# toposware/certificate-stark

Hardware: AMD Instinct MI355X
Metric: proofs/sec, state_transition AIR @ 2^20 steps (complete prove(): trace gen, LDE, Blake3 commitments, constraint evaluation, composition, DEEP, FRI, 96 queries) (higher is better)
Workload: dtype u64 (63-bit prime field, Montgomery) + u32 (Blake3)

## Files before the change

certificate-stark_amd/csrc/rounds_layout.h:

```cpp
#pragma once
#include "constraints.h"
#include "mds_mfma.cuh"

namespace cs {

struct RoundWindow { int reg, res_a, flag_a, res_b, flag_b; };
#define CS_ROUND_WINDOWS_INIT {{0, 0, 3, 0, -1}, {15, 14, 0, 15, 1}, {29, 28, 0, 29, 1}, {44, 42, 0, 44, 1}, {42, 42, 2, 0, -1}}
#define CS_WINDOW_GROUPS_INIT {{{0, 1, -1}, {-1, -1, -1}}, {{1, 2, 0}, {1, 2, 0}}, {{0, 2, -1}, {0, 2, -1}}, {{2, -1, -1}, {2, -1, -1}}, {{2, -1, -1}, {-1, -1, -1}}}

constexpr int RT_SECTIONS = 5 * 2 * 4;
constexpr int RT_A = 0, RT_UL = RT_SECTIONS * 64, RT_ML = RT_UL + RT_SECTIONS * 14 * 2, RT_MT = RT_ML + 14 * 14 * 2;
constexpr size_t MT_BYTES = (mdsmfma::table_bytes(14) + 15) & ~(size_t)15;
constexpr int RT_G = RT_MT + (int)(MT_BYTES / 8);
constexpr int RT_MF = (RT_G + RT_SECTIONS * 14 + 1) & ~1;

constexpr int MF_TILES_INV = 7, MF_TILES_SEC = 13, MF_KS_INV = 4, MF_KS_SEC = 7;
constexpr int MF_INV_D = RT_MF;
constexpr int MF_SEC_D = MF_INV_D + MF_TILES_INV * 4 * 8;
constexpr int MF_K = MF_SEC_D + MF_TILES_SEC * 4 * 16;
constexpr int RT_SIZE = MF_K + (14 + 2 * MF_TILES_SEC) * 4;
constexpr int RT_LAM = RT_SIZE;
static_assert(RT_LAM + CE_GFOLD_WORDS <= CE_RTAB_WORDS, "rtab size");
__host__ __device__ constexpr int mf_tile_base(int w) { return w == 0 ? 0 : w == 1 ? 2 : w == 2 ? 6 : w == 3 ? 10 : w == 4 ? 12 : 13; }
__host__ __device__ constexpr int mf_tile_window(int t) { return t < 2 ? 0 : t < 6 ? 1 : t < 10 ? 2 : t < 12 ? 3 : 4; }
__host__ __device__ constexpr int mf_tile_fs(int w, int local) { return (w == 1 || w == 2) ? local >> 1 : w == 3 ? local : 0; }
__host__ __device__ constexpr int mf_tile_pair(int w, int local) { return (w == 1 || w == 2) ? local & 1 : w == 0 ? local : 0; }

constexpr int MR_SECTIONS = 8, MR_A = 0, MR_UL = MR_SECTIONS * 64, MR_ML = MR_UL + MR_SECTIONS * 14 * 2, MR_G = MR_ML + 196 * 2;
constexpr int MRF_INV_D = MR_G + MR_SECTIONS * 14;
constexpr int MRF_SEC_D = MRF_INV_D + MF_TILES_INV * 32;
constexpr int MRF_K = MRF_SEC_D + 4 * 64;
constexpr int MR_SIZE = MRF_K + (14 + 8) * 4;
static_assert(MR_SIZE <= MERKLE_RTAB_LAMBDA, "MerkleAir rounds table");

hipError_t launch_merkle_rounds_mfma(const AirCombineParams &p, const uint64_t *ptab, uint64_t *d_rtab, unsigned nk, unsigned round_group, int which,
                                     hipStream_t stream);
hipError_t launch_rounds_mfma(const CeParams &p, uint64_t *d_even, hipStream_t stream);

}
```

certificate-stark_amd/csrc/rounds_mfma.hip:

```cpp
#include "rounds_layout.h"
#include "rescue.cuh"

namespace cs {
namespace {

using mdsmfma::v16i;
using mdsmfma::v4i;
typedef unsigned __int128 u128;

#ifndef RM_NT_
#define RM_NT_ 256
#endif
#ifndef RM_WAVES
#define RM_WAVES 2
#endif
constexpr int RM_NT = RM_NT_;
template <int PTS> constexpr int rw_rows = 32 * PTS + 2;
template <int PTS> constexpr int rw_img = 14 * rw_rows<PTS>;
constexpr uint64_t X0 = mdsmfma::X0;
constexpr uint64_t HALF_P = (FP_P - 1) / 2;
enum { P_SETUP = 0, P_HASH = 4, P_SCHNORR_HASH = 12, P_ARK = 20 };

__constant__ RoundWindow c_windows[5] = CS_ROUND_WINDOWS_INIT;
__constant__ int c_window_groups[5][2][3] = CS_WINDOW_GROUPS_INIT;

__device__ inline uint64_t digit_word(int64_t v) {
    uint64_t w = 0;
    int carry = 0;
    for (int a = 0; a < 8; a++) {
        int b = (a < 7 ? (int)(((uint64_t)v >> (8 * a)) & 0xff) : (int)(v >> 56)) + carry;
        carry = (a < 7 && b >= 128) ? 1 : 0;
        w |= (uint64_t)(uint8_t)(int8_t)(b - 256 * carry) << (8 * a);
    }
    return w;
}
__device__ __forceinline__ u128 acc0_offset() {
    u128 off = 0;
    for (int d = 0; d < 15; d++) off += (u128)mdsmfma::ACC0 << (8 * d);
    return off;
}

__device__ inline void build_inverse_tile(int T, int t, uint64_t *d_out, uint64_t *k_out) {
    if (t < 32) {
        const int g = t >> 4, h = (t >> 3) & 1, m = t & 7, i = 2 * T + g, j = 4 * (m >> 1) + 2 * h + (m & 1);
        d_out[(g * 2 + h) * 8 + m] = j < 14 ? digit_word((int64_t)c_inv_mds[i * 14 + j]) : 0;
    } else if (t < 34) {
        const int i = 2 * T + (t - 32);
        u128 k = 0;
        for (int j = 0; j < 14; j++) k += (u128)c_inv_mds[i * 14 + j] * X0;
        k -= acc0_offset();
        for (int q = 0; q < 4; q++) k_out[4 * (t - 32) + q] = (uint32_t)(k >> (32 * q));
    }
}
__device__ inline void build_section_tile(const fp *gam0, const fp *gam1, const uint32_t *ul0, const uint32_t *ul1, int t, uint64_t *d_out,
                                          uint64_t *k_out, fp (*csum)[32]) {
    if (t < 56) {
        const int g = t / 28, h = (t / 14) & 1, m = t % 14;
        fp c;
        if (m < 7) c = (g ? gam1 : gam0)[2 * m + h];
        else {
            const uint32_t *l = (g ? ul1 : ul0) + (2 * (m - 7) + h) * 4;
            c = fp_neg((fp)l[0] | ((fp)l[1] << 21) | ((fp)l[2] << 42));
        }
        d_out[(g * 2 + h) * 16 + m] = digit_word(c > HALF_P ? (int64_t)(c - FP_P) : (int64_t)c);
        csum[g][h * 14 + m] = c;
    } else {
        const int q = t - 56;
        d_out[(q >> 1) * 16 + 14 + (q & 1)] = 0;
    }
    __syncthreads();
    if (t < 2) {
        fp sum = 0;
        for (int e = 0; e < 28; e++) sum = fp_add(sum, csum[t][e]);
        const fp kc = fp_mul(fp_mul(X0 + HALF_P, sum), FP_R2);
        u128 k = (u128)kc + ((u128)(2 * FP_P) << 64);
        k -= acc0_offset();
        for (int q = 0; q < 4; q++) k_out[4 * t + q] = (uint32_t)(k >> (32 * q));
    }
}

__global__ void k_rounds_mfma_tables(fp *__restrict__ rtab) {
    rtab += (size_t)blockIdx.y * CE_RTAB_WORDS;
    const int t = threadIdx.x;
    if (blockIdx.x < MF_TILES_INV) {
        build_inverse_tile(blockIdx.x, t, rtab + MF_INV_D + blockIdx.x * 32, rtab + MF_K + 8 * blockIdx.x);
        return;
    }
    const int tile = blockIdx.x - MF_TILES_INV, w = mf_tile_window(tile), local = tile - mf_tile_base(w);
    const int sec = (w * 2 + mf_tile_fs(w, local)) * 4 + 2 * mf_tile_pair(w, local);
    __shared__ fp csum[2][32];
    const uint32_t *ul = (const uint32_t *)(rtab + RT_UL);
    build_section_tile(rtab + RT_G + sec * 14, rtab + RT_G + (sec + 1) * 14, ul + sec * 56, ul + (sec + 1) * 56, t, rtab + MF_SEC_D + tile * 64,
                       rtab + MF_K + 4 * (14 + 2 * tile), csum);
}
__global__ void k_merkle_rounds_mfma_tables(fp *__restrict__ rtab) {
    const int t = threadIdx.x;
    if (blockIdx.x < MF_TILES_INV) {
        build_inverse_tile(blockIdx.x, t, rtab + MRF_INV_D + blockIdx.x * 32, rtab + MRF_K + 8 * blockIdx.x);
        return;
    }
    const int w = blockIdx.x - MF_TILES_INV;
    __shared__ fp csum[2][32];
    const uint32_t *ul = (const uint32_t *)(rtab + MR_UL);
    build_section_tile(rtab + MR_G + (2 * w) * 14, rtab + MR_G + (2 * w + 1) * 14, ul + (2 * w) * 56, ul + (2 * w + 1) * 56, t, rtab + MRF_SEC_D + w * 64,
                       rtab + MRF_K + 4 * (14 + 2 * w), csum);
}

typedef __attribute__((address_space(3))) void lds_void;
typedef const __attribute__((address_space(1))) void glb_void;
template <int PTS>
__device__ __forceinline__ void fetch_window(const fp *rows, size_t n, int reg, int lane, fp *img) {
    if (lane < 16 * PTS + 1) {
#pragma unroll
        for (int j = 0; j < 14; j++)
            __builtin_amdgcn_global_load_lds((glb_void *)(rows + (size_t)(reg + j) * n), (lds_void *)(img + j * rw_rows<PTS>), 16, 0, 0);
    }
}
__device__ __forceinline__ v4i pack2(uint64_t a, uint64_t b) {
    v4i r;
    r[0] = (int)(uint32_t)a; r[1] = (int)(uint32_t)(a >> 32); r[2] = (int)(uint32_t)b; r[3] = (int)(uint32_t)(b >> 32);
    return r;
}
__device__ __forceinline__ v4i expand_frag(uint64_t d0, uint64_t d1, uint32_t sel_lo, uint32_t sel_hi) {
    v4i r;
    r[0] = (int)__builtin_amdgcn_perm((uint32_t)(d0 >> 32), (uint32_t)d0, sel_lo);
    r[1] = (int)__builtin_amdgcn_perm((uint32_t)(d0 >> 32), (uint32_t)d0, sel_hi);
    r[2] = (int)__builtin_amdgcn_perm((uint32_t)(d1 >> 32), (uint32_t)d1, sel_lo);
    r[3] = (int)__builtin_amdgcn_perm((uint32_t)(d1 >> 32), (uint32_t)d1, sel_hi);
    return r;
}
__device__ __forceinline__ v16i acc_start() {
    v16i a;
#pragma unroll
    for (int v = 0; v < 16; v++) a[v] = mdsmfma::ACC0;
    return a;
}
template <uint32_t V>
__device__ __forceinline__ uint32_t opaque_const() {
    uint32_t r;
    asm("s_mov_b32 %0, %1" : "=s"(r) : "n"(V));
    return r;
}
struct Shifts { uint32_t one, s8, s16, s24; };
__device__ __forceinline__ fp recombine_mad(const v16i &acc, const uint64_t (&k)[4], const Shifts &c) {
#ifdef RM_OLD_RECOMBINE
    return mdsmfma::recombine(acc, k[0] | (k[1] << 32), k[2] | (k[3] << 32));
#endif
    uint64_t s[4];
#pragma unroll
    for (int q = 0; q < 4; q++) {
        uint64_t t = mad_u64_u32((uint32_t)acc[4 * q], c.one, k[q]);
        t = mad_u64_u32((uint32_t)acc[4 * q + 1], c.s8, t);
        t = mad_u64_u32((uint32_t)acc[4 * q + 2], c.s16, t);
        if (4 * q + 3 < 15) t = mad_u64_u32((uint32_t)acc[4 * q + 3], c.s24, t);
        s[q] = t;
    }
    unsigned cy;
    const uint32_t w0 = (uint32_t)s[0];
    const uint32_t w1 = __builtin_addc((uint32_t)(s[0] >> 32), (uint32_t)s[1], 0u, &cy);
    const uint32_t w2 = __builtin_addc((uint32_t)(s[1] >> 32), (uint32_t)s[2], cy, &cy);
    const uint32_t w3 = (uint32_t)(s[2] >> 32) + (uint32_t)s[3] + cy;
    Acc128 a{((uint64_t)w1 << 32) | w0, ((uint64_t)w3 << 32) | w2};
    acc_fold(a);
    return acc_reduce(a);
}
#ifndef RM_DBUF
#define RM_DBUF 0
#endif
#ifndef RM_RESIDENT_
#define RM_RESIDENT_ 4096
#endif
constexpr unsigned RM_RESIDENT = RM_RESIDENT_;

struct Role {
    int lane, nn, h, ag;
    uint32_t sel_lo, sel_hi;
};
__device__ __forceinline__ void frag_selectors(int d, uint32_t &lo, uint32_t &hi) {
    lo = hi = 0;
#pragma unroll
    for (int b = 0; b < 4; b++) {
        const int a0 = d - b, a1 = d - 4 - b;
        lo |= (uint32_t)((a0 >= 0 && a0 <= 7 && d < 15) ? a0 : 0x0c) << (8 * b);
        hi |= (uint32_t)((a1 >= 0 && a1 <= 7 && d < 15) ? a1 : 0x0c) << (8 * b);
    }
}
__device__ __forceinline__ Role make_role(int lane) {
    Role r;
    r.lane = lane; r.nn = lane & 31; r.h = lane >> 5; r.ag = (r.nn >> 2) & 1;
    frag_selectors((r.nn & 3) + 4 * (r.nn >> 3), r.sel_lo, r.sel_hi);
    return r;
}
__device__ __forceinline__ void expand_inverse_table(v4i *inv_lds, const uint64_t *inv_d, int tid, int nthreads) {
    for (unsigned e = tid; e < MF_TILES_INV * MF_KS_INV * 64; e += nthreads) {
        const unsigned l = e & 63, ts = e >> 6, r = l & 31, hh = l >> 5, g = (r >> 2) & 1;
        uint32_t slo, shi;
        frag_selectors((int)((r & 3) + 4 * (r >> 3)), slo, shi);
        const uint64_t *dw = inv_d + ((ts >> 2) * 4 + g * 2 + hh) * 8 + 2 * (ts & 3);
        inv_lds[e] = expand_frag(dw[0], dw[1], slo, shi);
    }
}
template <int PTS, int DBUF>
__device__ __forceinline__ void window_operands(const fp *imgA, const fp *ark2, const v4i *inv_lds, const uint64_t *k_lds, const Role &ro,
                                                const Shifts &sh, v4i (&c)[PTS][MF_KS_SEC]) {
    constexpr int RWR = rw_rows<PTS>;
    const int h = ro.h, lane = ro.lane;
    v4i b[PTS][MF_KS_INV];
#pragma unroll
    for (int s = 0; s < MF_KS_INV; s++) {
        const int jb = (s == 3 && h) ? 12 : 4 * s + 2 * h;
        const fp k0 = ark2[jb], k1 = ark2[jb + 1];
#pragma unroll
        for (int pt = 0; pt < PTS; pt++)
            b[pt][s] = pack2(fp_sub(imgA[jb * RWR + 32 * pt + 1], k0) ^ X0, fp_sub(imgA[(jb + 1) * RWR + 32 * pt + 1], k1) ^ X0);
    }
    uint64_t held[PTS];
    auto inv_tile = [&](int T, v16i (&a)[PTS]) {
#pragma unroll
        for (int pt = 0; pt < PTS; pt++) a[pt] = acc_start();
#pragma unroll
        for (int s = 0; s < MF_KS_INV; s++) {
            const v4i fr = inv_lds[(T * MF_KS_INV + s) * 64 + lane];
#pragma unroll
            for (int pt = 0; pt < PTS; pt++) a[pt] = __builtin_amdgcn_mfma_i32_32x32x32_i8(fr, b[pt][s], a[pt], 0, 0, 0);
        }
    };
    auto finish_tile = [&](int T, const v16i (&a)[PTS]) {
        const uint64_t *kp = k_lds + 4 * (2 * T + h);
        const uint64_t kw[4] = {kp[0], kp[1], kp[2], kp[3]};
#pragma unroll
        for (int pt = 0; pt < PTS; pt++) {
            const uint64_t x = (fp_cube(recombine_mad(a[pt], kw, sh)) - HALF_P) ^ X0;
            if (T & 1) c[pt][T >> 1] = pack2(held[pt], x);
            else held[pt] = x;
        }
    };
    if constexpr (DBUF > 0) {
        v16i acc[2][PTS];
        inv_tile(0, acc[0]);
#pragma unroll
        for (int T = 0; T < MF_TILES_INV; T++) {
            if (T + 1 < MF_TILES_INV) inv_tile(T + 1, acc[(T + 1) & 1]);
            finish_tile(T, acc[T & 1]);
            if (T + 1 < MF_TILES_INV) {
#pragma unroll
                for (int e = 0; e < 4 * PTS; e++) {
                    __builtin_amdgcn_sched_group_barrier(0x008, 1, 0);
                    __builtin_amdgcn_sched_group_barrier(0x002, DBUF, 0);
                }
            }
        }
    } else {
#pragma unroll
        for (int T = 0; T < MF_TILES_INV; T++) {
            v16i acc[PTS];
            inv_tile(T, acc);
            finish_tile(T, acc);
        }
    }
#pragma unroll
    for (int t = 0; t < 7; t++) {
#pragma unroll
        for (int pt = 0; pt < PTS; pt++) {
            const uint64_t x = (fp_cube(imgA[(2 * t + h) * RWR + 32 * pt]) - HALF_P) ^ X0;
            if (t & 1) held[pt] = x;
            else c[pt][3 + (t >> 1)] = pack2(held[pt], x);
        }
    }
}
template <int PTS>
__device__ __forceinline__ void section_tile(const uint64_t *tile_d, const uint64_t *kp, const Role &ro, const Shifts &sh, const v4i (&c)[PTS][MF_KS_SEC],
                                             fp (&r)[PTS]) {
    v16i a[PTS];
#pragma unroll
    for (int pt = 0; pt < PTS; pt++) a[pt] = acc_start();
    const uint64_t *dw = tile_d + (ro.ag * 2 + ro.h) * 16;
#pragma unroll
    for (int s = 0; s < MF_KS_SEC; s++) {
        const v4i fr = expand_frag(dw[2 * s], dw[2 * s + 1], ro.sel_lo, ro.sel_hi);
#pragma unroll
        for (int pt = 0; pt < PTS; pt++) a[pt] = __builtin_amdgcn_mfma_i32_32x32x32_i8(fr, c[pt][s], a[pt], 0, 0, 0);
    }
    const uint64_t kw[4] = {kp[0], kp[1], kp[2], kp[3]};
#pragma unroll
    for (int pt = 0; pt < PTS; pt++) r[pt] = recombine_mad(a[pt], kw, sh);
}
__device__ __forceinline__ fp other_half(fp v) {
    const uint32_t lo = __shfl_xor((uint32_t)v, 32), hi = __shfl_xor((uint32_t)(v >> 32), 32);
    return ((uint64_t)hi << 32) | lo;
}

#ifndef RM_DBUF1
#define RM_DBUF1 0
#endif
#ifndef RM_PTS
#define RM_PTS 2
#endif
constexpr size_t RM_LDS_INV = (size_t)MF_TILES_INV * MF_KS_INV * 64 * 16;
template <int PTS, int NT = RM_NT> constexpr size_t rm_lds_img = (size_t)(NT / 64) * rw_img<PTS> * 8;
constexpr size_t RM_LDS_SEC = (size_t)MF_TILES_SEC * 4 * 16 * 8;
constexpr size_t RM_LDS_KINV = 14 * 32, RM_LDS_KSEC = (size_t)2 * MF_TILES_SEC * 32;
constexpr size_t RM_LDS_ARK = 8 * 14 * 8, RM_LDS_ATAB = (size_t)2 * MF_TILES_SEC * 8 * 8;
template <int PTS, int M, int NT> constexpr size_t rm_lds = RM_LDS_INV + rm_lds_img<PTS, NT> + RM_LDS_KINV + RM_LDS_ARK + M * (RM_LDS_SEC + RM_LDS_KSEC + RM_LDS_ATAB);

template <int PTS, int M, int NT>
__global__ __launch_bounds__(NT, PTS == 1 ? 3 : RM_WAVES) void k_rounds_mfma(CeParams p, fp *__restrict__ out) {
    constexpr int RWR = rw_rows<PTS>, WROWS = 32 * PTS, BROWS = NT / 64 * WROWS;
    constexpr int RM_NT = NT;
    extern __shared__ __attribute__((aligned(16))) uint8_t lds[];
    v4i *inv_lds = (v4i *)lds;
    fp *img_all = (fp *)(lds + RM_LDS_INV);
    uint64_t *kinv_lds = (uint64_t *)(lds + RM_LDS_INV + rm_lds_img<PTS, NT>);
    fp *ark2_lds = kinv_lds + RM_LDS_KINV / 8;
    uint64_t *secd_lds = ark2_lds + RM_LDS_ARK / 8;
    uint64_t *ksec_lds = secd_lds + M * (RM_LDS_SEC / 8);
    fp *atab_lds = ksec_lds + M * (RM_LDS_KSEC / 8);

    const size_t n = (size_t)1 << p.log_n;
    const unsigned kk = 2 * blockIdx.y, kc = (p.k0 >> 1) + blockIdx.y, ka = 2 * kc;
    const int tid = threadIdx.x, lane = tid & 63;
    const Role ro = make_role(lane);
    const int nn = ro.nn, h = ro.h;
    const fp *rt = p.rtab;
    expand_inverse_table(inv_lds, rt + MF_INV_D, tid, RM_NT);
    for (unsigned e = tid; e < RM_LDS_KINV / 8; e += RM_NT) kinv_lds[e] = rt[MF_K + e];
    for (unsigned e = tid; e < M * (RM_LDS_SEC / 8); e += RM_NT) secd_lds[e] = rt[(size_t)(e / (RM_LDS_SEC / 8)) * CE_RTAB_WORDS + MF_SEC_D + e % (RM_LDS_SEC / 8)];
    for (unsigned e = tid; e < M * (RM_LDS_KSEC / 8); e += RM_NT) ksec_lds[e] = rt[(size_t)(e / (RM_LDS_KSEC / 8)) * CE_RTAB_WORDS + MF_K + 14 * 4 + e % (RM_LDS_KSEC / 8)];
    if (tid < 8 * 14) {
        const unsigned r = tid / 14, c = tid % 14;
        ark2_lds[tid] = p.ptab[((size_t)ka * 48 + P_ARK + 14 + c) * 1024 + r];
    }
    for (unsigned e = tid; e < M * 2 * MF_TILES_SEC * 8; e += RM_NT) {
        const int c = e / (2 * MF_TILES_SEC * 8), r = e % (2 * MF_TILES_SEC * 8), tile = r >> 4, g = (r >> 3) & 1, w = mf_tile_window(tile), local = tile - mf_tile_base(w);
        const int sec = (w * 2 + mf_tile_fs(w, local)) * 4 + 2 * mf_tile_pair(w, local) + g;
        atab_lds[e] = rt[(size_t)c * CE_RTAB_WORDS + RT_A + sec * 64 + ka * 8 + (r & 7)];
    }
    __syncthreads();

    fp *img = img_all + (size_t)(tid >> 6) * rw_img<PTS>;
    const uint64_t *k_lds = kinv_lds;
    const fp *imgA = img + nn;
    const unsigned jrp = (unsigned)(nn & 7);
    const fp *ark2 = ark2_lds + jrp * 14;
    const fp *per = p.ptab + (size_t)(p.k0 + kk) * 48 * 1024;
    const fp *colbase = p.lde + (size_t)kk * 94 * n;
    const Shifts sh{opaque_const<1>(), opaque_const<1u << 8>(), opaque_const<1u << 16>(), opaque_const<1u << 24>()};
    const size_t nblk = n / BROWS;
    size_t blk = blockIdx.x;
    auto rows_of = [&](size_t b) {
        const size_t jw = b * (size_t)BROWS + (size_t)(tid >> 6) * WROWS;
        return colbase + jw + 2 * lane - ((lane == 16 * PTS && jw + WROWS == n) ? n : 0);
    };
    const fp *rows = rows_of(blk);
    if (blk < nblk) fetch_window<PTS>(rows, n, c_windows[0].reg, lane, img);
#pragma unroll 1
    for (; blk < nblk; blk += gridDim.x) {
        const size_t jw = blk * (size_t)BROWS + (size_t)(tid >> 6) * WROWS;
        fp fl[PTS][3];
#pragma unroll
        for (int pt = 0; pt < PTS; pt++) {
            const size_t r = (jw + nn + 32 * pt) & 1023;
            fl[pt][0] = per[(size_t)P_SETUP * 1024 + r]; fl[pt][1] = per[(size_t)P_HASH * 1024 + r]; fl[pt][2] = per[(size_t)P_SCHNORR_HASH * 1024 + r];
        }
        fp sm[M][PTS][5];
#pragma unroll
        for (int c = 0; c < M; c++)
#pragma unroll
            for (int pt = 0; pt < PTS; pt++)
#pragma unroll
                for (int q = 0; q < 5; q++) sm[c][pt][q] = 0;
#pragma unroll 1
        for (int wdx = 0; wdx < 5; wdx++) {
            const RoundWindow w = c_windows[wdx];
            asm volatile("s_waitcnt vmcnt(0)" ::: "memory");
            v4i c[PTS][MF_KS_SEC];
            window_operands<PTS, PTS == 1 ? RM_DBUF1 : RM_DBUF>(imgA, ark2, inv_lds, k_lds, ro, sh, c);
            asm volatile("s_waitcnt lgkmcnt(0)" ::: "memory");
#ifndef RM_EXP_NODMA
            if (wdx < 4) fetch_window<PTS>(rows, n, c_windows[wdx + 1].reg, lane, img);
            else if (blk + gridDim.x < nblk) { rows = rows_of(blk + gridDim.x); fetch_window<PTS>(rows, n, c_windows[0].reg, lane, img); }
#endif
#pragma unroll
            for (int cs = 0; cs < M; cs++) {
                fp x[PTS][2];
#pragma unroll
                for (int pt = 0; pt < PTS; pt++) x[pt][0] = x[pt][1] = 0;
#ifdef RM_EXP_NOSEC
                const int t0 = 0, t1 = 0;
                x[0][0] = (fp)c[0][0][0] ^ (fp)c[0][6][3];
#else
                const int t0 = mf_tile_base(wdx), t1 = mf_tile_base(wdx + 1);
#endif
#pragma unroll 1
                for (int tile = t0; tile < t1; tile++) {
                    const int local = tile - t0, fs = mf_tile_fs(wdx, local), u = mf_tile_pair(wdx, local);
                    fp r[PTS];
                    section_tile<PTS>(secd_lds + (cs * MF_TILES_SEC + tile) * 64, ksec_lds + 4 * (cs * 2 * MF_TILES_SEC + 2 * tile + h), ro, sh, c, r);
                    const fp at = atab_lds[(cs * 2 * MF_TILES_SEC + 2 * tile + h) * 8 + jrp];
                    const int fg = fs ? w.flag_b : w.flag_a;
#pragma unroll
                    for (int pt = 0; pt < PTS; pt++) {
                        const fp f = fg == 0 ? fl[pt][0] : fg == 1 ? fl[pt][1] : fg == 2 ? fl[pt][2] : fp_add(fl[pt][0], fl[pt][1]);
                        const fp v = fp_mul(f, fp_sub(r[pt], at));
                        if (u) x[pt][1] = fp_add(x[pt][1], v);
                        else x[pt][0] = fp_add(x[pt][0], v);
                    }
                }
#pragma unroll
                for (int pt = 0; pt < PTS; pt++) {
                    if (wdx == 0 || wdx == 2) sm[cs][pt][0] = fp_add(sm[cs][pt][0], x[pt][0]);
                    else if (wdx == 1) sm[cs][pt][1] = fp_add(sm[cs][pt][1], x[pt][0]);
                    else sm[cs][pt][2] = fp_add(sm[cs][pt][2], x[pt][0]);
                    if (wdx == 0) sm[cs][pt][3] = fp_add(sm[cs][pt][3], x[pt][1]);
                    else if (wdx < 3) sm[cs][pt][4] = fp_add(sm[cs][pt][4], x[pt][1]);
                }
            }
        }
#pragma unroll
        for (int cs = 0; cs < M; cs++) {
            fp tot[PTS][4];
#pragma unroll
            for (int pt = 0; pt < PTS; pt++) {
                const fp s012 = fp_add(fp_add(sm[cs][pt][0], sm[cs][pt][1]), sm[cs][pt][2]), s34 = fp_add(sm[cs][pt][3], sm[cs][pt][4]);
                tot[pt][0] = h ? 0 : s012; tot[pt][1] = h ? fp_add(sm[cs][pt][0], s34) : 0;
                tot[pt][2] = h ? sm[cs][pt][1] : sm[cs][pt][3]; tot[pt][3] = h ? sm[cs][pt][2] : sm[cs][pt][4];
            }
            fp *o = out + (size_t)cs * CE_SPLIT_TABLES * 4 * n;
            if constexpr (PTS == 2) {
                const size_t j = jw + lane;
#pragma unroll
                for (int q = 0; q < 4; q++) {
                    const fp mine = h ? tot[1][q] : tot[0][q], give = h ? tot[0][q] : tot[1][q];
                    o[((size_t)q * 4 + kc) * n + j] = fp_add(mine, other_half(give));
                }
            } else {
                const size_t j = jw + nn;
#pragma unroll
                for (int e = 0; e < 2; e++) {
                    const fp got = other_half(h ? tot[0][e] : tot[0][2 + e]);
                    const int q = 2 * h + e;
                    o[((size_t)q * 4 + kc) * n + j] = fp_add(h ? tot[0][2 + e] : tot[0][e], got);
                }
            }
        }
    }
}

constexpr size_t MRM_LDS_SEC = 4 * 64 * 8, MRM_LDS_K = (14 + 8) * 32, MRM_LDS_ATAB = MR_SECTIONS * 8 * 8;
constexpr size_t MRM_LDS = RM_LDS_INV + rm_lds_img<2> + MRM_LDS_SEC + MRM_LDS_K + RM_LDS_ARK + MRM_LDS_ATAB;
struct MerkleRoundsParams {
    const fp *lde, *w;
    fp *out;
    fp xshift[8];
    uint64_t xadj;
    uint32_t log_n, k0, stride;
};
template <int W0, int NWIN, int WIDTH, int PCOLS, int FLAGCOL, int ARKCOL, bool ADD>
__global__ __launch_bounds__(RM_NT, RM_WAVES) void k_merkle_rounds_mfma(MerkleRoundsParams p, const fp *__restrict__ ptab, const fp *__restrict__ rtab) {
    extern __shared__ __attribute__((aligned(16))) uint8_t lds[];
    v4i *inv_lds = (v4i *)lds;
    fp *img_all = (fp *)(lds + RM_LDS_INV);
    uint64_t *secd_lds = (uint64_t *)(lds + RM_LDS_INV + rm_lds_img<2>);
    uint64_t *k_lds = secd_lds + MRM_LDS_SEC / 8;
    fp *ark2_lds = k_lds + MRM_LDS_K / 8;
    fp *atab_lds = ark2_lds + RM_LDS_ARK / 8;

    const size_t n = (size_t)1 << p.log_n;
    const unsigned kk = blockIdx.y, k = p.k0 + kk;
    if (k % p.stride) return;
    const int tid = threadIdx.x, lane = tid & 63;
    const Role ro = make_role(lane);
    const int nn = ro.nn, h = ro.h;
    expand_inverse_table(inv_lds, rtab + MRF_INV_D, tid, RM_NT);
    for (unsigned e = tid; e < NWIN * 64; e += RM_NT) secd_lds[e] = rtab[MRF_SEC_D + e];
    for (unsigned e = tid; e < (14 + 2 * NWIN) * 4; e += RM_NT) k_lds[e] = rtab[MRF_K + e];
    if (tid < 8 * 14) {
        const unsigned r = tid / 14, c = tid % 14;
        ark2_lds[tid] = ptab[((size_t)k * PCOLS + ARKCOL + 14 + c) * 512 + r];
    }
    if (tid < MR_SECTIONS * 8) atab_lds[tid] = rtab[MR_A + (tid >> 3) * 64 + k * 8 + (tid & 7)];
    __syncthreads();

    fp *img = img_all + (size_t)(tid >> 6) * rw_img<2>;
    const fp *imgA = img + nn;
    const unsigned jrp = (unsigned)(nn & 7);
    const fp *ark2 = ark2_lds + jrp * 14;
    const fp *colbase = p.lde + (size_t)kk * WIDTH * n;
    const Shifts sh{opaque_const<1>(), opaque_const<1u << 8>(), opaque_const<1u << 16>(), opaque_const<1u << 24>()};
    const size_t nblk = n / RM_NT;
    size_t blk = blockIdx.x;
    auto rows_of = [&](size_t b) {
        const size_t jw = b * (size_t)RM_NT + (size_t)(tid >> 6) * 64;
        return colbase + jw + 2 * lane - ((lane == 32 && jw + 64 == n) ? n : 0);
    };
    const fp *rows = rows_of(blk);
    if (blk < nblk) fetch_window<2>(rows, n, c_windows[W0].reg, lane, img);
#pragma unroll 1
    for (; blk < nblk; blk += gridDim.x) {
        const size_t j = blk * (size_t)RM_NT + (size_t)(tid >> 6) * 64 + lane;
        fp tA = 0, tB = 0;
#pragma unroll 1
        for (int wdx = 0; wdx < NWIN; wdx++) {
            asm volatile("s_waitcnt vmcnt(0)" ::: "memory");
            v4i c[2][MF_KS_SEC];
            window_operands<2, 0>(imgA, ark2, inv_lds, k_lds, ro, sh, c);
            asm volatile("s_waitcnt lgkmcnt(0)" ::: "memory");
            if (wdx + 1 < NWIN) fetch_window<2>(rows, n, c_windows[W0 + wdx + 1].reg, lane, img);
            else if (blk + gridDim.x < nblk) { rows = rows_of(blk + gridDim.x); fetch_window<2>(rows, n, c_windows[W0].reg, lane, img); }
            __builtin_amdgcn_sched_barrier(0);
            fp r[2];
            section_tile<2>(secd_lds + wdx * 64, k_lds + 4 * (14 + 2 * wdx + h), ro, sh, c, r);
            const fp at = atab_lds[(2 * wdx + h) * 8 + jrp];
            tA = fp_add(tA, fp_sub(r[0], at));
            tB = fp_add(tB, fp_sub(r[1], at));
        }
        const fp got = other_half(h ? tA : tB);
        const fp ta = h ? got : tA, tb = h ? tB : got;
        const fp flag = ptab[((size_t)k * PCOLS + FLAGCOL) * 512 + (j & 511)];
        const fp xp = fp_mul(p.xshift[k], p.w[(j * p.xadj) & (n - 1)]);
        const fp v = fp_mul(flag, fp_add(ta, fp_mul(xp, tb)));
        fp *o = p.out + (size_t)kk * n + j;
        *o = ADD ? fp_add(*o, v) : v;
    }
}

}

template <int PTS, int M, int NT>
static hipError_t launch_rounds_mfma_as(const CeParams &p, uint64_t *d_even, hipStream_t stream) {
    const size_t n = (size_t)1 << p.log_n;
    constexpr int BROWS = NT / 64 * 32 * PTS;
    constexpr size_t LDS = rm_lds<PTS, M, NT>;
    if (n % BROWS) return hipErrorInvalidValue;
    static const hipError_t attr = hipFuncSetAttribute((const void *)k_rounds_mfma<PTS, M, NT>, hipFuncAttributeMaxDynamicSharedMemorySize, (int)LDS);
    if (attr != hipSuccess) return attr;
    hipLaunchKernelGGL(k_rounds_mfma_tables, dim3(MF_TILES_INV + MF_TILES_SEC, M), dim3(64), 0, stream, p.rtab);
    const unsigned ny = p.nkc ? p.nkc : 4, nblk = (unsigned)(n / BROWS), gx = RM_RESIDENT / ny < nblk ? RM_RESIDENT / ny : nblk;
    hipLaunchKernelGGL((k_rounds_mfma<PTS, M, NT>), dim3(gx, ny), dim3(NT), LDS, stream, p, d_even);
    return hipGetLastError();
}
hipError_t launch_rounds_mfma(const CeParams &p, uint64_t *d_even, hipStream_t stream) {
    const unsigned m = p.m ? p.m : 1;
    if (m == 1) return launch_rounds_mfma_as<RM_PTS, 1, RM_NT>(p, d_even, stream);
    if (m == 2) return launch_rounds_mfma_as<2, 2, 256>(p, d_even, stream);
    if (m == 3) return launch_rounds_mfma_as<2, 3, 512>(p, d_even, stream);
    return hipErrorInvalidValue;
}

hipError_t launch_merkle_rounds_mfma(const AirCombineParams &p, const uint64_t *ptab, uint64_t *d_rtab, unsigned nk, unsigned round_group, int which,
                                     hipStream_t stream) {
    const size_t n = (size_t)1 << p.log_n;
    if (n % RM_NT) return hipErrorInvalidValue;
    const unsigned nblk = (unsigned)(n / RM_NT), gx = RM_RESIDENT / nk ? (RM_RESIDENT / nk < nblk ? RM_RESIDENT / nk : nblk) : 1;
    if (round_group >= AIR_MAX_GROUPS) return hipErrorInvalidValue;
    MerkleRoundsParams q;
    q.lde = p.lde; q.w = p.w; q.out = p.out; q.xadj = p.tgrp_adj[round_group]; q.log_n = p.log_n; q.k0 = p.k0; q.stride = p.stride;
    for (int k = 0; k < 8; k++) q.xshift[k] = p.tgrp_shift[k][round_group];
    if (which == 0) {
        auto kern = k_merkle_rounds_mfma<0, 4, 65, 33, 4, 5, false>;
        static const hipError_t attr = hipFuncSetAttribute((const void *)kern, hipFuncAttributeMaxDynamicSharedMemorySize, (int)MRM_LDS);
        if (attr != hipSuccess) return attr;
        hipLaunchKernelGGL(k_merkle_rounds_mfma_tables, dim3(MF_TILES_INV + 4), dim3(64), 0, stream, d_rtab);
        hipLaunchKernelGGL(kern, dim3(gx, nk), dim3(RM_NT), MRM_LDS, stream, q, ptab, (const fp *)d_rtab);
    } else {
        auto kern = k_merkle_rounds_mfma<4, 1, 56, 36, 7, 8, true>;
        static const hipError_t attr = hipFuncSetAttribute((const void *)kern, hipFuncAttributeMaxDynamicSharedMemorySize, (int)MRM_LDS);
        if (attr != hipSuccess) return attr;
        hipLaunchKernelGGL(k_merkle_rounds_mfma_tables, dim3(MF_TILES_INV + 1), dim3(64), 0, stream, d_rtab);
        hipLaunchKernelGGL(kern, dim3(gx, nk), dim3(RM_NT), MRM_LDS, stream, q, ptab, (const fp *)d_rtab);
    }
    return hipGetLastError();
}

}
```

Baseline: 43.33.

## Precompute inverse-MDS MFMA tables at compile time using residue-folded recombination

Moves construction of the inverse-MDS MFMA fragment tables and recombination constants into a constexpr builder placed in device memory. This removes the per-launch inverse-tile table blocks and the in-kernel fragment expansion; kernels now copy the tables straight into LDS. The tables pre-multiply coefficients by 2^32 and pack two outputs per tile (4 tiles instead of 7), so recombination becomes a residue/Montgomery-style fold with a single conditional subtraction. The risk is correctness of the new digit bounds and reduction, and more constant data that each block loads.

```diff
diff --git a/certificate-stark_amd/csrc/rounds_layout.h b/certificate-stark_amd/csrc/rounds_layout.h
--- a/certificate-stark_amd/csrc/rounds_layout.h
+++ b/certificate-stark_amd/csrc/rounds_layout.h
@@ -14,11 +14,10 @@
 constexpr int RT_G = RT_MT + (int)(MT_BYTES / 8);
 constexpr int RT_MF = (RT_G + RT_SECTIONS * 14 + 1) & ~1;
 
-constexpr int MF_TILES_INV = 7, MF_TILES_SEC = 13, MF_KS_INV = 4, MF_KS_SEC = 7;
-constexpr int MF_INV_D = RT_MF;
-constexpr int MF_SEC_D = MF_INV_D + MF_TILES_INV * 4 * 8;
+constexpr int MF_TILES_INV = 4, MF_TILES_SEC = 13, MF_KS_INV = 4, MF_KS_SEC = 7;
+constexpr int MF_SEC_D = RT_MF;
 constexpr int MF_K = MF_SEC_D + MF_TILES_SEC * 4 * 16;
-constexpr int RT_SIZE = MF_K + (14 + 2 * MF_TILES_SEC) * 4;
+constexpr int RT_SIZE = MF_K + 2 * MF_TILES_SEC * 4;
 constexpr int RT_LAM = RT_SIZE;
 static_assert(RT_LAM + CE_GFOLD_WORDS <= CE_RTAB_WORDS, "rtab size");
 __host__ __device__ constexpr int mf_tile_base(int w) { return w == 0 ? 0 : w == 1 ? 2 : w == 2 ? 6 : w == 3 ? 10 : w == 4 ? 12 : 13; }
@@ -27,10 +26,9 @@
 __host__ __device__ constexpr int mf_tile_pair(int w, int local) { return (w == 1 || w == 2) ? local & 1 : w == 0 ? local : 0; }
 
 constexpr int MR_SECTIONS = 8, MR_A = 0, MR_UL = MR_SECTIONS * 64, MR_ML = MR_UL + MR_SECTIONS * 14 * 2, MR_G = MR_ML + 196 * 2;
-constexpr int MRF_INV_D = MR_G + MR_SECTIONS * 14;
-constexpr int MRF_SEC_D = MRF_INV_D + MF_TILES_INV * 32;
+constexpr int MRF_SEC_D = MR_G + MR_SECTIONS * 14;
 constexpr int MRF_K = MRF_SEC_D + 4 * 64;
-constexpr int MR_SIZE = MRF_K + (14 + 8) * 4;
+constexpr int MR_SIZE = MRF_K + 8 * 4;
 static_assert(MR_SIZE <= MERKLE_RTAB_LAMBDA, "MerkleAir rounds table");
 
 hipError_t launch_merkle_rounds_mfma(const AirCombineParams &p, const uint64_t *ptab, uint64_t *d_rtab, unsigned nk, unsigned round_group, int which,
diff --git a/certificate-stark_amd/csrc/rounds_mfma.hip b/certificate-stark_amd/csrc/rounds_mfma.hip
--- a/certificate-stark_amd/csrc/rounds_mfma.hip
+++ b/certificate-stark_amd/csrc/rounds_mfma.hip
@@ -1,4 +1,5 @@
 #include "rounds_layout.h"
+#include "rounds_residue.h"
 #include "rescue.cuh"
 
 namespace cs {
@@ -20,6 +21,10 @@
 constexpr uint64_t X0 = mdsmfma::X0;
 constexpr uint64_t HALF_P = (FP_P - 1) / 2;
 enum { P_SETUP = 0, P_HASH = 4, P_SCHNORR_HASH = 12, P_ARK = 20 };
+
+static_assert(rresidue::P == FP_P && rresidue::P1 == FP_P1 && rresidue::X0 == X0 && rresidue::ACC0 == mdsmfma::ACC0, "rounds_residue.h: constants");
+static_assert(rresidue::TILES == MF_TILES_INV && rresidue::KSTEPS == MF_KS_INV, "rounds_residue.h: tile counts");
+__device__ const rresidue::Tables c_residue = rresidue::build_tables(rresidue::INV_MDS_CAN);
 
 __constant__ RoundWindow c_windows[5] = CS_ROUND_WINDOWS_INIT;
 __constant__ int c_window_groups[5][2][3] = CS_WINDOW_GROUPS_INIT;
@@ -40,18 +45,6 @@
     return off;
 }
 
-__device__ inline void build_inverse_tile(int T, int t, uint64_t *d_out, uint64_t *k_out) {
-    if (t < 32) {
-        const int g = t >> 4, h = (t >> 3) & 1, m = t & 7, i = 2 * T + g, j = 4 * (m >> 1) + 2 * h + (m & 1);
-        d_out[(g * 2 + h) * 8 + m] = j < 14 ? digit_word((int64_t)c_inv_mds[i * 14 + j]) : 0;
-    } else if (t < 34) {
-        const int i = 2 * T + (t - 32);
-        u128 k = 0;
-        for (int j = 0; j < 14; j++) k += (u128)c_inv_mds[i * 14 + j] * X0;
-        k -= acc0_offset();
-        for (int q = 0; q < 4; q++) k_out[4 * (t - 32) + q] = (uint32_t)(k >> (32 * q));
-    }
-}
 __device__ inline void build_section_tile(const fp *gam0, const fp *gam1, const uint32_t *ul0, const uint32_t *ul1, int t, uint64_t *d_out,
                                           uint64_t *k_out, fp (*csum)[32]) {
     if (t < 56) {
@@ -82,28 +75,19 @@
 __global__ void k_rounds_mfma_tables(fp *__restrict__ rtab) {
     rtab += (size_t)blockIdx.y * CE_RTAB_WORDS;
     const int t = threadIdx.x;
-    if (blockIdx.x < MF_TILES_INV) {
-        build_inverse_tile(blockIdx.x, t, rtab + MF_INV_D + blockIdx.x * 32, rtab + MF_K + 8 * blockIdx.x);
-        return;
-    }
-    const int tile = blockIdx.x - MF_TILES_INV, w = mf_tile_window(tile), local = tile - mf_tile_base(w);
+    const int tile = blockIdx.x, w = mf_tile_window(tile), local = tile - mf_tile_base(w);
     const int sec = (w * 2 + mf_tile_fs(w, local)) * 4 + 2 * mf_tile_pair(w, local);
     __shared__ fp csum[2][32];
     const uint32_t *ul = (const uint32_t *)(rtab + RT_UL);
     build_section_tile(rtab + RT_G + sec * 14, rtab + RT_G + (sec + 1) * 14, ul + sec * 56, ul + (sec + 1) * 56, t, rtab + MF_SEC_D + tile * 64,
-                       rtab + MF_K + 4 * (14 + 2 * tile), csum);
+                       rtab + MF_K + 8 * tile, csum);
 }
 __global__ void k_merkle_rounds_mfma_tables(fp *__restrict__ rtab) {
-    const int t = threadIdx.x;
-    if (blockIdx.x < MF_TILES_INV) {
-        build_inverse_tile(blockIdx.x, t, rtab + MRF_INV_D + blockIdx.x * 32, rtab + MRF_K + 8 * blockIdx.x);
-        return;
-    }
-    const int w = blockIdx.x - MF_TILES_INV;
+    const int t = threadIdx.x, w = blockIdx.x;
     __shared__ fp csum[2][32];
     const uint32_t *ul = (const uint32_t *)(rtab + MR_UL);
     build_section_tile(rtab + MR_G + (2 * w) * 14, rtab + MR_G + (2 * w + 1) * 14, ul + (2 * w) * 56, ul + (2 * w + 1) * 56, t, rtab + MRF_SEC_D + w * 64,
-                       rtab + MRF_K + 4 * (14 + 2 * w), csum);
+                       rtab + MRF_K + 8 * w, csum);
 }
 
 typedef __attribute__((address_space(3))) void lds_void;
@@ -141,7 +125,7 @@
     asm("s_mov_b32 %0, %1" : "=s"(r) : "n"(V));
     return r;
 }
-struct Shifts { uint32_t one, s8, s16, s24; };
+using rresidue::Shifts;
 __device__ __forceinline__ fp recombine_mad(const v16i &acc, const uint64_t (&k)[4], const Shifts &c) {
 #ifdef RM_OLD_RECOMBINE
     return mdsmfma::recombine(acc, k[0] | (k[1] << 32), k[2] | (k[3] << 32));
@@ -164,6 +148,12 @@
     acc_fold(a);
     return acc_reduce(a);
 }
+template <int SLOT>
+__device__ __forceinline__ fp recombine_residue(const v16i &acc, uint64_t k0, uint64_t k1, const Shifts &c) {
+    const uint32_t d[8] = {(uint32_t)acc[8 * SLOT], (uint32_t)acc[8 * SLOT + 1], (uint32_t)acc[8 * SLOT + 2], (uint32_t)acc[8 * SLOT + 3],
+                           (uint32_t)acc[8 * SLOT + 4], (uint32_t)acc[8 * SLOT + 5], (uint32_t)acc[8 * SLOT + 6], (uint32_t)acc[8 * SLOT + 7]};
+    return fp_reduce_once(rresidue::recombine(d, k0, k1, c));
+}
 #ifndef RM_DBUF
 #define RM_DBUF 0
 #endif
@@ -191,14 +181,10 @@
     frag_selectors((r.nn & 3) + 4 * (r.nn >> 3), r.sel_lo, r.sel_hi);
     return r;
 }
-__device__ __forceinline__ void expand_inverse_table(v4i *inv_lds, const uint64_t *inv_d, int tid, int nthreads) {
-    for (unsigned e = tid; e < MF_TILES_INV * MF_KS_INV * 64; e += nthreads) {
-        const unsigned l = e & 63, ts = e >> 6, r = l & 31, hh = l >> 5, g = (r >> 2) & 1;
-        uint32_t slo, shi;
-        frag_selectors((int)((r & 3) + 4 * (r >> 3)), slo, shi);
-        const uint64_t *dw = inv_d + ((ts >> 2) * 4 + g * 2 + hh) * 8 + 2 * (ts & 3);
-        inv_lds[e] = expand_frag(dw[0], dw[1], slo, shi);
-    }
+__device__ __forceinline__ void load_inverse_table(v4i *inv_lds, uint64_t *kinv_lds, int tid, int nthreads) {
+    const v4i *src = (const v4i *)c_residue.frag;
+    for (unsigned e = tid; e < MF_TILES_INV * MF_KS_INV * 64; e += nthreads) inv_lds[e] = src[e];
+    for (unsigned e = tid; e < rresidue::OUTPUTS * 2; e += nthreads) kinv_lds[e] = c_residue.k[e >> 1][e & 1];
 }
 template <int PTS, int DBUF>
 __device__ __forceinline__ void window_operands(const fp *imgA, const fp *ark2, const v4i *inv_lds, const uint64_t *k_lds, const Role &ro,
@@ -226,12 +212,12 @@
         }
     };
     auto finish_tile = [&](int T, const v16i (&a)[PTS]) {
-        const uint64_t *kp = k_lds + 4 * (2 * T + h);
-        const uint64_t kw[4] = {kp[0], kp[1], kp[2], kp[3]};
+        const uint64_t *kp = k_lds + 2 * rresidue::output_of(T, h, 0);
+        const uint64_t k00 = kp[0], k01 = kp[1];
 #pragma unroll
         for (int pt = 0; pt < PTS; pt++) {
-            const uint64_t x = (fp_cube(recombine_mad(a[pt], kw, sh)) - HALF_P) ^ X0;
-            if (T & 1) c[pt][T >> 1] = pack2(held[pt], x);
+            const uint64_t x = (fp_cube(recombine_residue<0>(a[pt], k00, k01, sh)) - HALF_P) ^ X0;
+            if (T + 1 < MF_TILES_INV) c[pt][T] = pack2(x, (fp_cube(recombine_residue<1>(a[pt], kp[4], kp[5], sh)) - HALF_P) ^ X0);
             else held[pt] = x;
         }
     };
@@ -299,7 +285,7 @@
 constexpr size_t RM_LDS_INV = (size_t)MF_TILES_INV * MF_KS_INV * 64 * 16;
 template <int PTS, int NT = RM_NT> constexpr size_t rm_lds_img = (size_t)(NT / 64) * rw_img<PTS> * 8;
 constexpr size_t RM_LDS_SEC = (size_t)MF_TILES_SEC * 4 * 16 * 8;
-constexpr size_t RM_LDS_KINV = 14 * 32, RM_LDS_KSEC = (size_t)2 * MF_TILES_SEC * 32;
+constexpr size_t RM_LDS_KINV = 14 * 16, RM_LDS_KSEC = (size_t)2 * MF_TILES_SEC * 32;
 constexpr size_t RM_LDS_ARK = 8 * 14 * 8, RM_LDS_ATAB = (size_t)2 * MF_TILES_SEC * 8 * 8;
 template <int PTS, int M, int NT> constexpr size_t rm_lds = RM_LDS_INV + rm_lds_img<PTS, NT> + RM_LDS_KINV + RM_LDS_ARK + M * (RM_LDS_SEC + RM_LDS_KSEC + RM_LDS_ATAB);
 
@@ -322,10 +308,9 @@
     const Role ro = make_role(lane);
     const int nn = ro.nn, h = ro.h;
     const fp *rt = p.rtab;
-    expand_inverse_table(inv_lds, rt + MF_INV_D, tid, RM_NT);
-    for (unsigned e = tid; e < RM_LDS_KINV / 8; e += RM_NT) kinv_lds[e] = rt[MF_K + e];
+    load_inverse_table(inv_lds, kinv_lds, tid, RM_NT);
     for (unsigned e = tid; e < M * (RM_LDS_SEC / 8); e += RM_NT) secd_lds[e] = rt[(size_t)(e / (RM_LDS_SEC / 8)) * CE_RTAB_WORDS + MF_SEC_D + e % (RM_LDS_SEC / 8)];
-    for (unsigned e = tid; e < M * (RM_LDS_KSEC / 8); e += RM_NT) ksec_lds[e] = rt[(size_t)(e / (RM_LDS_KSEC / 8)) * CE_RTAB_WORDS + MF_K + 14 * 4 + e % (RM_LDS_KSEC / 8)];
+    for (unsigned e = tid; e < M * (RM_LDS_KSEC / 8); e += RM_NT) ksec_lds[e] = rt[(size_t)(e / (RM_LDS_KSEC / 8)) * CE_RTAB_WORDS + MF_K + e % (RM_LDS_KSEC / 8)];
     if (tid < 8 * 14) {
         const unsigned r = tid / 14, c = tid % 14;
         ark2_lds[tid] = p.ptab[((size_t)ka * 48 + P_ARK + 14 + c) * 1024 + r];
@@ -446,7 +431,7 @@
     }
 }
 
-constexpr size_t MRM_LDS_SEC = 4 * 64 * 8, MRM_LDS_K = (14 + 8) * 32, MRM_LDS_ATAB = MR_SECTIONS * 8 * 8;
+constexpr size_t MRM_LDS_SEC = 4 * 64 * 8, MRM_LDS_K = RM_LDS_KINV + 8 * 32, MRM_LDS_ATAB = MR_SECTIONS * 8 * 8;
 constexpr size_t MRM_LDS = RM_LDS_INV + rm_lds_img<2> + MRM_LDS_SEC + MRM_LDS_K + RM_LDS_ARK + MRM_LDS_ATAB;
 struct MerkleRoundsParams {
     const fp *lde, *w;
@@ -462,6 +447,7 @@
     fp *img_all = (fp *)(lds + RM_LDS_INV);
     uint64_t *secd_lds = (uint64_t *)(lds + RM_LDS_INV + rm_lds_img<2>);
     uint64_t *k_lds = secd_lds + MRM_LDS_SEC / 8;
+    uint64_t *ksec_lds = k_lds + RM_LDS_KINV / 8;
     fp *ark2_lds = k_lds + MRM_LDS_K / 8;
     fp *atab_lds = ark2_lds + RM_LDS_ARK / 8;
 
@@ -471,9 +457,9 @@
     const int tid = threadIdx.x, lane = tid & 63;
     const Role ro = make_role(lane);
     const int nn = ro.nn, h = ro.h;
-    expand_inverse_table(inv_lds, rtab + MRF_INV_D, tid, RM_NT);
+    load_inverse_table(inv_lds, k_lds, tid, RM_NT);
     for (unsigned e = tid; e < NWIN * 64; e += RM_NT) secd_lds[e] = rtab[MRF_SEC_D + e];
-    for (unsigned e = tid; e < (14 + 2 * NWIN) * 4; e += RM_NT) k_lds[e] = rtab[MRF_K + e];
+    for (unsigned e = tid; e < 2 * NWIN * 4; e += RM_NT) ksec_lds[e] = rtab[MRF_K + e];
     if (tid < 8 * 14) {
         const unsigned r = tid / 14, c = tid % 14;
         ark2_lds[tid] = ptab[((size_t)k * PCOLS + ARKCOL + 14 + c) * 512 + r];
@@ -509,7 +495,7 @@
             else if (blk + gridDim.x < nblk) { rows = rows_of(blk + gridDim.x); fetch_window<2>(rows, n, c_windows[W0].reg, lane, img); }
             __builtin_amdgcn_sched_barrier(0);
             fp r[2];
-            section_tile<2>(secd_lds + wdx * 64, k_lds + 4 * (14 + 2 * wdx + h), ro, sh, c, r);
+            section_tile<2>(secd_lds + wdx * 64, ksec_lds + 4 * (2 * wdx + h), ro, sh, c, r);
             const fp at = atab_lds[(2 * wdx + h) * 8 + jrp];
             tA = fp_add(tA, fp_sub(r[0], at));
             tB = fp_add(tB, fp_sub(r[1], at));
@@ -534,7 +520,7 @@
     if (n % BROWS) return hipErrorInvalidValue;
     static const hipError_t attr = hipFuncSetAttribute((const void *)k_rounds_mfma<PTS, M, NT>, hipFuncAttributeMaxDynamicSharedMemorySize, (int)LDS);
     if (attr != hipSuccess) return attr;
-    hipLaunchKernelGGL(k_rounds_mfma_tables, dim3(MF_TILES_INV + MF_TILES_SEC, M), dim3(64), 0, stream, p.rtab);
+    hipLaunchKernelGGL(k_rounds_mfma_tables, dim3(MF_TILES_SEC, M), dim3(64), 0, stream, p.rtab);
     const unsigned ny = p.nkc ? p.nkc : 4, nblk = (unsigned)(n / BROWS), gx = RM_RESIDENT / ny < nblk ? RM_RESIDENT / ny : nblk;
     hipLaunchKernelGGL((k_rounds_mfma<PTS, M, NT>), dim3(gx, ny), dim3(NT), LDS, stream, p, d_even);
     return hipGetLastError();
@@ -560,13 +546,13 @@
         auto kern = k_merkle_rounds_mfma<0, 4, 65, 33, 4, 5, false>;
         static const hipError_t attr = hipFuncSetAttribute((const void *)kern, hipFuncAttributeMaxDynamicSharedMemorySize, (int)MRM_LDS);
         if (attr != hipSuccess) return attr;
-        hipLaunchKernelGGL(k_merkle_rounds_mfma_tables, dim3(MF_TILES_INV + 4), dim3(64), 0, stream, d_rtab);
+        hipLaunchKernelGGL(k_merkle_rounds_mfma_tables, dim3(4), dim3(64), 0, stream, d_rtab);
         hipLaunchKernelGGL(kern, dim3(gx, nk), dim3(RM_NT), MRM_LDS, stream, q, ptab, (const fp *)d_rtab);
     } else {
         auto kern = k_merkle_rounds_mfma<4, 1, 56, 36, 7, 8, true>;
         static const hipError_t attr = hipFuncSetAttribute((const void *)kern, hipFuncAttributeMaxDynamicSharedMemorySize, (int)MRM_LDS);
         if (attr != hipSuccess) return attr;
-        hipLaunchKernelGGL(k_merkle_rounds_mfma_tables, dim3(MF_TILES_INV + 1), dim3(64), 0, stream, d_rtab);
+        hipLaunchKernelGGL(k_merkle_rounds_mfma_tables, dim3(1), dim3(64), 0, stream, d_rtab);
         hipLaunchKernelGGL(kern, dim3(gx, nk), dim3(RM_NT), MRM_LDS, stream, q, ptab, (const fp *)d_rtab);
     }
     return hipGetLastError();
diff --git a/certificate-stark_amd/csrc/rounds_residue.h b/certificate-stark_amd/csrc/rounds_residue.h
--- /dev/null
+++ b/certificate-stark_amd/csrc/rounds_residue.h
@@ -0,0 +1,129 @@
+#pragma once
+#include <stdint.h>
+#include "constants_gen.h"
+
+namespace cs {
+namespace rresidue {
+
+typedef unsigned __int128 u128;
+
+constexpr uint64_t P = 0x4180000000000001ULL;
+constexpr uint32_t P1 = 0x41800000u;
+constexpr uint64_t X0 = 0x0080808080808080ULL;
+constexpr int ACC0 = 1 << 23;
+constexpr int TILES = 4, KSTEPS = 4, OUTPUTS = 14;
+constexpr int FRAG_WORDS = TILES * KSTEPS * 64 * 2;
+
+constexpr uint64_t INV_MDS_CAN[196] = CS_INV_MDS_CAN_INIT;
+
+constexpr int output_of(int T, int g, int slot) { return 4 * T + 2 * slot + g; }
+constexpr int row_half(int r) { return (r >> 2) & 1; }
+constexpr int row_reg(int r) { return (r & 3) + 4 * (r >> 3); }
+
+constexpr uint64_t add_mod(uint64_t a, uint64_t b) { return a + b >= P ? a + b - P : a + b; }
+constexpr uint64_t shl_mod(uint64_t v, int bits) {
+    for (int k = 0; k < bits; k++) v = add_mod(v, v);
+    return v;
+}
+constexpr uint64_t digit_word(uint64_t v) {
+    uint64_t w = 0;
+    int carry = 0;
+    for (int a = 0; a < 8; a++) {
+        const int b = (int)((v >> (8 * a)) & 0xff) + carry;
+        carry = b >= 128 ? 1 : 0;
+        w |= (uint64_t)((b - 256 * carry) & 0xff) << (8 * a);
+    }
+    return w;
+}
+constexpr int digit_of(uint64_t word, int a) { const int b = (int)((word >> (8 * a)) & 0xff); return b >= 128 ? b - 256 : b; }
+
+struct Tables {
+    alignas(16) uint64_t frag[FRAG_WORDS];
+    uint64_t k[16][2];
+};
+
+constexpr Tables build_tables(const uint64_t (&m_can)[196]) {
+    Tables t = {};
+    for (int i = 0; i < OUTPUTS; i++) {
+        const int T = i >> 2, slot = (i >> 1) & 1, g = i & 1;
+        uint64_t sum = 0;
+        for (int j = 0; j < 14; j++) {
+            const int s = j >> 2, hh = (j >> 1) & 1, e = j & 1;
+            uint64_t rho = shl_mod(m_can[i * 14 + j], 32);
+            for (int b = 0; b < 8; b++) {
+                if (b < 7) sum = add_mod(sum, rho);
+                const uint64_t dw = digit_word(rho);
+                for (int a = 0; a < 8; a++) {
+                    const int v = 8 * slot + a, r = (v & 3) + 8 * (v >> 2) + 4 * g;
+                    t.frag[((T * KSTEPS + s) * 64 + 32 * hh + r) * 2 + e] |= ((dw >> (8 * a)) & 0xff) << (8 * b);
+                }
+                rho = shl_mod(rho, 8);
+            }
+        }
+        const uint64_t off = shl_mod(0x0101010101010101ULL, 23);
+        const uint64_t k = add_mod(shl_mod(sum, 7), P - off);
+        t.k[i][0] = k & 0xffffffffULL;
+        t.k[i][1] = (k >> 32) + P1 + 1;
+    }
+    return t;
+}
+
+struct Shifts { uint32_t one, s8, s16, s24; };
+#if defined(__HIP_DEVICE_COMPILE__)
+#define RR_HD __host__ __device__ __forceinline__
+#define RR_KEEP(x) asm("" : "+v"(x))
+#elif defined(__HIPCC__)
+#define RR_HD __host__ __device__ inline
+#define RR_KEEP(x)
+#else
+#define RR_HD inline
+#define RR_KEEP(x)
+#endif
+RR_HD uint64_t recombine(const uint32_t (&acc)[8], uint64_t k0, uint64_t k1, const Shifts &sh) {
+    uint64_t s0 = (uint64_t)acc[0] * sh.one + k0;
+    RR_KEEP(s0);
+    s0 = (uint64_t)acc[1] * sh.s8 + s0;
+    s0 = (uint64_t)acc[2] * sh.s16 + s0;
+    s0 = (uint64_t)acc[3] * sh.s24 + s0;
+    RR_KEEP(s0);
+    uint64_t s1 = (uint64_t)acc[4] * sh.one + k1;
+    RR_KEEP(s1);
+    s1 = (uint64_t)acc[5] * sh.s8 + s1;
+    s1 = (uint64_t)acc[6] * sh.s16 + s1;
+    s1 = (uint64_t)acc[7] * sh.s24 + s1;
+    RR_KEEP(s1);
+    uint64_t hi = (uint64_t)(uint32_t)(s0 >> 32) * sh.one + s1;
+    RR_KEEP(hi);
+    return (uint64_t)(~(uint32_t)s0) * P1 + hi;
+}
+#undef RR_KEEP
+#undef RR_HD
+constexpr uint64_t reduce_once(uint64_t r) { return r >= P ? r - P : r; }
+
+constexpr int table_digit(const Tables &t, int T, int r, int k) {
+    const int s = k >> 5, hh = (k >> 4) & 1, e = (k >> 3) & 1, b = k & 7;
+    return digit_of(t.frag[((T * KSTEPS + s) * 64 + 32 * hh + r) * 2 + e], b);
+}
+constexpr int64_t row_abs_bound(const Tables &t, int T, int r) {
+    int64_t sum = 0;
+    for (int k = 0; k < 128; k++) { const int d = table_digit(t, T, r, k); sum += (d < 0 ? -d : d) * 128; }
+    return sum;
+}
+constexpr int64_t acc_extreme(const Tables &t, int T, int r, bool upper) {
+    int64_t v = ACC0;
+    for (int k = 0; k < 128; k++) {
+        const int d = table_digit(t, T, r, k), lo = (k & 7) < 7 ? -128 : 0, hi = (k & 7) < 7 ? 127 : 0x41;
+        v += d * ((d > 0) == upper ? hi : lo);
+    }
+    return v;
+}
+constexpr int output_row(int i, int a) { const int v = 8 * ((i >> 1) & 1) + a; return (v & 3) + 8 * (v >> 2) + 4 * (i & 1); }
+constexpr u128 v_max(const Tables &t, int i) {
+    u128 v = ((u128)(t.k[i][1] - P1 - 1) << 32) + t.k[i][0];
+    for (int a = 0; a < 8; a++) v += (u128)acc_extreme(t, i >> 2, output_row(i, a), true) << (8 * a);
+    return v;
+}
+constexpr u128 redc_max(const Tables &t, int i) { return (v_max(t, i) >> 32) + P; }
+
+}
+}
```

Result: no change. 43.89 (median of 6 runs) (+1.3%).
